# johannes-graeter/limo

Measured on AMD Instinct MI355X. Metric: keyframe-BA window solves/sec (5 KF, ~2k landmarks), higher is better.
Workload: dtype f64; 1 GPU; C2: KITTI-00-shaped windows, 5 keyframes x 2000 landmarks, LiDAR depth + ground plane, solveTrimmed schedule {2, trim 5%, <=100 LM iterations}; batch_windows_per_gpu=16384, distinct_windows_per_gpu=4096, observations_per_batch=144288124, depth_observations_per_batch=68405568, parallelism=single, converged=16328

## Files before the change

### limo_amd/csrc/kba_buffers.hpp

```cpp
#pragma once
#include <algorithm>
#include <cstddef>
#include <vector>

#include "kba_pack.hpp"

namespace kba {

template <typename F>
void for_each_buffer(const PackedBatch& P, BatchView& bv, F f) {
    bv.n_win = P.n_win;
    bv.TK = P.TK;
    bv.TL = P.TL;
    bv.TO = P.TO;
    bv.TV = P.TV;
    bv.TG = P.TG;
    bv.n_blk = P.n_blk;
    bv.n_lblk = P.n_lblk;
    bv.n_sblk = P.n_sblk;
    bv.Vmax = P.Vmax;
    bv.SO = P.SO;
    bv.SL = P.SL;
    bv.SG = P.SG;
    bv.SD = P.SD;
// ... 9 lines not shown
    KBA_BUF(win, NW * sizeof(WinDesc), P.win.data());
    KBA_BUF(st, NW * sizeof(WinState), nullptr);
    KBA_BUF(red, NW * sizeof(WinRed), nullptr);
    KBA_BUF(pose, TK * 7 * D, P.pose.data());
    KBA_BUF(pdir, TK * 3 * D, P.pdir.data());
    KBA_BUF(pdist, TK * D, P.pdist.data());
    KBA_BUF(lm, TL * 3 * D, P.lm.data());
    KBA_BUF(pose_c, TK * 7 * D, P.pose.data());
    KBA_BUF(pdir_c, TK * 3 * D, P.pdir.data());
    KBA_BUF(pdist_c, TK * D, P.pdist.data());
    KBA_BUF(lm_c, TL * 3 * D, P.lm.data());
    KBA_BUF(kf_win, TK * I, P.kf_win.data());
    KBA_BUF(kf_blk0, TK * I, P.kf_blk0.data());
    KBA_BUF(kf_nblk, TK * I, P.kf_nblk.data());
    KBA_BUF(kf_gp0, TK * I, P.kf_gp0.data());
    KBA_BUF(kf_ngp, TK * I, P.kf_ngp.data());
    KBA_BUF(cmask, TK * kCamSlots, P.cmask.data());
    KBA_BUF(cpresent, TK * kCamSlots, P.cpresent.data());
    KBA_BUF(cslot, TK * kCamSlots * I, P.cslot.data());
    KBA_BUF(lm_win, TL * I, P.lm_win.data());
    KBA_BUF(lm_id, TL * I, P.lm_id.data());
    KBA_BUF(lm_weight, TL * D, P.lm_weight.data());
    KBA_BUF(lm_state, TL, P.lm_state.data());
    KBA_BUF(lm_gp, TL * I, P.lm_gp.data());
    KBA_BUF(lm_slot, P.lm_slot.size() * I, P.lm_slot.data());
    KBA_BUF(view_kf, TV * I, P.view_kf.data());
    KBA_BUF(view_win, TV * I, P.view_win.data());
    KBA_BUF(view_cam, TV * 16 * D, P.view_cam.data());
    KBA_BUF(view_lin, TV * kViewLin * D, nullptr);
    KBA_BUF(view_lin_c, TV * kViewLin * D, nullptr);
    KBA_BUF(blk_view, NB * I, P.blk_view.data());
    KBA_BUF(blk_obs0, NB * I, P.blk_obs0.data());
    KBA_BUF(blk_n, NB * I, P.blk_n.data());
    KBA_BUF(obs_lm, TO * I, P.obs_lm.data());
    KBA_BUF(obs_u, TO * sizeof(float), P.obs_u.data());
    KBA_BUF(obs_v, TO * sizeof(float), P.obs_v.data());
    KBA_BUF(obs_d, TO * sizeof(float), P.obs_d.data());
    KBA_BUF(lblk_win, NL * I, P.lblk_win.data());
    KBA_BUF(lblk_lm0, NL * I, P.lblk_lm0.data());
    KBA_BUF(lblk_n, NL * I, P.lblk_n.data());
    KBA_BUF(sblk_win, NS * I, P.sblk_win.data());
    KBA_BUF(sblk_lm0, NS * I, P.sblk_lm0.data());
    KBA_BUF(sblk_n, NS * I, P.sblk_n.data());
    KBA_BUF(sgrp, NS * sizeof(SchurGroup), P.sgrp.empty() ? nullptr : P.sgrp.data());
    KBA_BUF(gp_lm, TG * I, P.gp_lm.data());
    KBA_BUF(gp_kf, TG * I, P.gp_kf.data());
    KBA_BUF(gp_w, TG * D, P.gp_w.data());
    KBA_BUF(gp_r, (size_t)P.SG * D, nullptr);
    KBA_BUF(gp_F, (size_t)P.SG * 10 * D, nullptr);
    KBA_BUF(gp_E, (size_t)P.SG * 3 * D, nullptr);
    KBA_BUF(gp_cost, TG * D, nullptr);
    KBA_BUF(gp_cost_c, TG * D, nullptr);
    KBA_BUF(obs_r, (size_t)(P.evaluate_only ? P.SO * 2 + P.SD : 1) * D, nullptr);
    KBA_BUF(obs_c, (size_t)(P.evaluate_only ? 1 : P.SO * 2) * D, nullptr);
    KBA_BUF(obs_Jp, (size_t)(P.evaluate_only ? P.SO * 12 + P.SD * 6 : 1) * D, nullptr);
    KBA_BUF(obs_Jl, (size_t)(P.evaluate_only ? P.SO * 6 + P.SD * 3 : 1) * D, nullptr);
    if (P.evaluate_only) KBA_BUF(echunk, (size_t)std::max(1, P.n_echunk) * sizeof(EvalChunk), P.echunk.empty() ? nullptr : P.echunk.data());
    KBA_BUF(lv_part, (size_t)(P.lvpart_total > 0 ? P.lvpart_total : 1) * D, nullptr);
    KBA_BUF(lblk_linfail, NL * D, nullptr);
    KBA_BUF(lm_V, (size_t)P.SL * 6 * D, nullptr);
    KBA_BUF(lm_g, (size_t)P.SL * 3 * D, nullptr);
    KBA_BUF(lm_scale, (size_t)P.SL * 3 * D, nullptr);
    KBA_BUF(lm_Li, (size_t)P.SL * 6 * D, nullptr);
    KBA_BUF(lblk_part, NL * 8 * D, nullptr);
    KBA_BUF(Hcc, (size_t)(P.hcc_total > 0 ? P.hcc_total : 1) * D, nullptr);
    KBA_BUF(gc, TK * kCamSlots * D, nullptr);
    KBA_BUF(scale_c, TK * kCamSlots * D, nullptr);
    KBA_BUF(yc, TK * kCamSlots * D, nullptr);
    KBA_BUF(delta_c, TK * kCamSlots * D, nullptr);
    KBA_BUF(S_part, (size_t)(P.spart_total > 0 ? P.spart_total : 1) * D, nullptr);
    KBA_BUF(S_red, (size_t)(P.sred_total > 0 ? P.sred_total : 1) * D, nullptr);
    KBA_BUF(cam_scratch, (size_t)(P.camscr_total > 0 ? P.camscr_total : 1) * D, nullptr);
    KBA_BUF(reg_cost, NW * 2 * D, nullptr);
    KBA_BUF(trim_rep, TL * D, nullptr);
    KBA_BUF(trim_dep, TL * D, nullptr);
    KBA_BUF(n_active, 8 * I, nullptr);
    if (P.n_shards > 1) {
        KBA_BUF(lblk_owner, NL * I, P.lblk_owner.data());
        KBA_BUF(gp_owner, TG * I, P.gp_owner.data());
    }
#undef KBA_BUF
}

inline ExchangeLayout exchange_layout(const PackedBatch& P) {
    ExchangeLayout L;
    auto pad = [](size_t n) { return (n + 31) / 32 * 32; };
    L.P = P.n_shards;
    L.n_win = P.n_win;
    L.TK = P.TK;
    L.n_lv = pad((size_t)std::max<int64_t>(1, P.xlv_total));
    L.n_w = pad((size_t)std::max(1, P.n_win));
    L.n_gp = pad((size_t)std::max(1, P.TK) * kGpRed);
    L.n_lb = pad((size_t)std::max(1, P.n_win) * 8);
    L.n_S = pad((size_t)std::max<int64_t>(1, P.sred_total / std::max(1, P.n_shards)));
    size_t o = 0;
    L.b_lv = o, o += L.n_lv;
    L.b_lf = o, o += L.n_w;
    L.b_gp = o, o += L.n_gp;
    L.b_gc = o, o += L.n_w;
    L.b_gcc = o, o += L.n_w;
    L.b_lb = o, o += L.n_lb;
    L.b_S = o, o += L.n_S;
    L.b_total = o;
    const size_t Pn = (size_t)L.P;
    o = 0;
    L.c_lv = o, o += Pn * L.n_lv;
    L.c_lf = o, o += Pn * L.n_w;
// ... 49 lines not shown
```

### limo_amd/csrc/kba_items.hpp

```cpp
#pragma once
#include "kba_layout.hpp"
#include "kba_lm.hpp"
#include "kba_math.hpp"

#ifndef KBA_SYNC
#define KBA_SYNC() ((void)0)
#endif
#if defined(KBA_PROFILE_TICKS) && defined(__HIPCC__)
__device__ long long kba_ticks[2][24];
#endif
#if defined(KBA_PROFILE_TICKS) && defined(__HIP_DEVICE_COMPILE__)
#define KBA_TICK(n)                                                                   \
    do {                                                                              \
        if (w == 0 && (tid == 0 || tid == nt - 1)) kba_ticks[tid != 0][n] = clock64(); \
    } while (0)
#else
#define KBA_TICK(n) ((void)0)
#endif

namespace kba {

struct LinLane {
    double e[kLinPartial];
    int fail;
// ... 270 lines not shown
        a.g[2] += e2 * r3[row];
    }
}
struct LmTailIn {
    int gg;
    int compute_scale;
    double radius;
    double sc[3];
};
KBA_HD void lin_lm_tail_fetch(const BatchView& bv, int w, int gl, LmTailIn& t) {
    t.gg = bv.lm_gp[gl];
    t.compute_scale = bv.st[w].compute_scale;
    t.radius = bv.st[w].radius;
    for (int i = 0; i < 3; ++i) t.sc[i] = t.compute_scale ? 1.0 : bv.lm_scale[i * bv.SL + gl];
}
KBA_HD void lin_lm_finish(const BatchView& bv, const SolveConsts& c, int gl, const double* x, const LmTailIn& t, LmAcc& a, double* part) {
    double* V = a.V;
    double* g = a.g;
    const int gg = t.gg;
    if (gg >= 0) {
        const double e0 = bv.gp_E[0 * bv.SG + gg], e1 = bv.gp_E[1 * bv.SG + gg], e2 = bv.gp_E[2 * bv.SG + gg];
        const double r = bv.gp_r[gg];
        V[0] += e0 * e0;
        V[1] += e0 * e1;
        V[2] += e0 * e2;
        V[3] += e1 * e1;
        V[4] += e1 * e2;
        V[5] += e2 * e2;
        g[0] += e0 * r;
        g[1] += e1 * r;
        g[2] += e2 * r;
    }
    for (int i = 0; i < 6; ++i) bv.lm_V[i * bv.SL + gl] = V[i];
    for (int i = 0; i < 3; ++i) bv.lm_g[i * bv.SL + gl] = g[i];
    double sc[3];
    if (t.compute_scale) {
        const double d[3] = {V[0], V[3], V[5]};
        for (int i = 0; i < 3; ++i) bv.lm_scale[i * bv.SL + gl] = sc[i] = c.jacobi_scaling ? 1.0 / (1.0 + sqrt(d[i])) : 1.0;
    } else {
        for (int i = 0; i < 3; ++i) sc[i] = t.sc[i];
    }
    part[0] = fmax(fabs(g[0]), fmax(fabs(g[1]), fabs(g[2])));
    part[1] = x[0] * x[0] + x[1] * x[1] + x[2] * x[2];
    part[5] = lm_damp_store(bv, c, t.radius, gl, sc, V, g) ? 1.0 : 0.0;
}
KBA_HD int lin_lm_lane(const BatchView& bv, const SolveConsts& c, int w, int gl, bool want_cost, LinLane* cam, double* part) {
    const WinDesc& wd = bv.win[w];
    part[0] = part[1] = part[5] = 0.0;
    for (int j = 0; j < wd.n_view; ++j) {
        cam[j].fail = 0;
        for (int i = 0; i < kLinPartial; ++i) cam[j].e[i] = 0.0;
    }
    const int state = bv.lm_state[gl];
    if (state == 0) return 0;
    LmAcc acc;
    for (int i = 0; i < 6; ++i) acc.V[i] = 0.0;
    for (int i = 0; i < 3; ++i) acc.g[i] = 0.0;
    int fail = 0;
    for (int j = 0; j < wd.n_view; ++j) {
        const int s = bv.lm_slot[(int64_t)j * bv.SL + gl];
        if (s < 0) continue;
        LinIn in;
        lin_fetch(bv, s, gl, in);
        const double* vl = bv.view_lin + (int64_t)kViewLin * (wd.view0 + j);
        double r3[3], c4[4];
        if (j < wd.n_view_fixed0) {
            if (!lin_obs<false>(vl, c, in, want_cost, r3, c4, cam[j])) fail = 1;
            if (state == 2) {
                cam[j].e[kLinFixedCost] = cam[j].e[0];
                cam[j].e[0] = 0.0;
            }
        } else {
            if (!lin_obs<true>(vl, c, in, want_cost, r3, c4, cam[j])) fail = 1;
            bv.obs_c[s] = c4[0];
            bv.obs_c[bv.SO + s] = c4[3];
        }
        lin_lm_accum(vl, r3, c4, acc);
    }
    if (state == 1) {
        LmTailIn t;
        lin_lm_tail_fetch(bv, w, gl, t);
        lin_lm_finish(bv, c, gl, bv.lm + 3 * (int64_t)gl, t, acc, part);
    }
    return fail;
}

KBA_HD void trim_residual_lane(const BatchView& bv, int b, int t, double* plane_rep, double* plane_dep) {
    if (t >= bv.blk_n[b]) return;
    const int view = bv.blk_view[b];
    const int64_t o = bv.blk_obs0[b] + t;
    const int gl = bv.obs_lm[o];
    double nr = -1.0, nd = -1.0;
    if (bv.lm_state[gl]) {
        const double* cam = bv.view_cam + 16 * (int64_t)view;
        double ruv[2], rd, zc[3];
        if (obs_residual(bv.pose + 7 * (int64_t)bv.view_kf[view], cam + 4, cam + 13, cam[0], cam[1], cam[2],
                         bv.lm + 3 * (int64_t)gl, bv.obs_u[o], bv.obs_v[o], bv.obs_d[o], ruv, &rd, zc)) {
            nr = sqrt(ruv[0] * ruv[0] + ruv[1] * ruv[1]);
        } else {
            nr = INFINITY;
        }
        if (bv.obs_d[o] > 0.0f) nd = fabs(zc[2] - static_cast<double>(bv.obs_d[o]));
    }
    plane_rep[o] = nr;
    plane_dep[o] = nd;
}

KBA_HD bool gp_row_fixed(const BatchView& bv, int g) {
    return bv.lm_state[bv.gp_lm[g]] == 2 && !bv.cmask[(int64_t)bv.gp_kf[g] * kCamSlots];
}
KBA_HD void gp_lane(const BatchView& bv, int g, bool candidate, double* cost_out) {
    const int gl = bv.gp_lm[g];
    const int gk = bv.gp_kf[g];
    GpOut o;
    const int state = bv.lm_state[gl];
    if (!state) {
        if (!candidate) {
            bv.gp_r[g] = 0.0;
            for (int i = 0; i < 10; ++i) bv.gp_F[i * bv.SG + g] = 0.0;
            for (int i = 0; i < 3; ++i) bv.gp_E[i * bv.SG + g] = 0.0;
        }
        cost_out[g] = 0.0;
        return;
    }
    if (candidate) {
        if (state == 2 && !bv.cmask[(int64_t)gk * kCamSlots]) {
            cost_out[g] = 0.0;
            return;
// ... 65 lines not shown
    double GB[9];
#pragma unroll
    for (int i = 0; i < 3; ++i) {
        GB[i * 3 + 0] = G[i * 3] * b00;
        GB[i * 3 + 1] = G[i * 3] * b01 + G[i * 3 + 1] * b11;
        GB[i * 3 + 2] = G[i * 3] * b02 + G[i * 3 + 1] * b12 + G[i * 3 + 2] * b22;
    }
#pragma unroll
    for (int a = 0; a < 3; ++a) {
#pragma unroll
        for (int cc = 0; cc < 3; ++cc) {
            const double yr = sc6[a] * (M[a] * GB[cc] + M[3 + a] * GB[3 + cc] + M[6 + a] * GB[6 + cc]);
            const double yt = sc6[3 + a] * GB[a * 3 + cc];
            Y[a * 3 + cc] = ASSIGN ? yr : Y[a * 3 + cc] + yr;
            Y[(3 + a) * 3 + cc] = ASSIGN ? yt : Y[(3 + a) * 3 + cc] + yt;
        }
    }
}

KBA_HD void schur_gp_block(const BatchView& bv, int gg, const uint8_t* cm, const double* lmk, const double* sc10, double* Y) {
    double E[3];
#pragma unroll
    for (int i = 0; i < 3; ++i) E[i] = bv.gp_E[i * bv.SG + gg];
    const double y0 = E[0] * lmk[0], y1 = E[0] * lmk[1] + E[1] * lmk[2], y2 = E[0] * lmk[3] + E[1] * lmk[4] + E[2] * lmk[5];
#pragma unroll
    for (int a = 0; a < kCamSlots; ++a) {
        if (!cm[a]) continue;
        const double f = bv.gp_F[a * bv.SG + gg] * sc10[a];
        Y[a * 3 + 0] += f * y0;
        Y[a * 3 + 1] += f * y1;
        Y[a * 3 + 2] += f * y2;
    }
}

KBA_HD void schur_pair_block(const BatchView& bv, const WinDesc& wd, int gl, int kl, const double* lmk, const double* sc,
                             const int* vkl, bool with_plane, double* Y) {
    for (int i = 0; i < 3 * kCamSlots; ++i) Y[i] = 0.0;
    const int row0 = kl * kCamSlots;
    const uint8_t* cm = bv.cmask + (int64_t)wd.cam0 + row0;
    if (cm[0]) {
        const double* pose = bv.pose + 7 * (int64_t)(wd.kf0 + kl);
        double R[9], M[9];
        bool have = false;
        for (int j = 0; j < wd.n_view; ++j) {
            if (vkl[j] != kl) continue;
            const int s = bv.lm_slot[(int64_t)j * bv.SL + gl];
            if (s < 0) continue;
            if (!have) {
                quat_R(pose, R);
                rot_tangent_from_R(R, quat_norm2_minus_1(pose), bv.lm + 3 * (int64_t)gl, M);
                have = true;
            }
            double Ft[9], c4[4];
            c4[0] = bv.obs_c[s];
            c4[3] = bv.obs_c[bv.SO + s];
            view_xy(bv.view_lin + (int64_t)kViewLin * (wd.view0 + j), bv.lm + 3 * (int64_t)gl, &c4[1], &c4[2]);
            ft_build(c4, bv.view_cam + 16 * (int64_t)(wd.view0 + j) + 4, Ft);
            schur_pose_block(Ft, R, M, lmk, sc + row0, Y);
        }
    }
    if (!with_plane) return;
    const int gg = bv.lm_gp[gl];
    if (gg < 0 || bv.gp_kf[gg] - wd.kf0 != kl) return;
    schur_gp_block(bv, gg, cm, lmk, sc + row0, Y);
}

KBA_HD void schur_load_lm(const BatchView& bv, int gl, double* lmk) {
#pragma unroll
    for (int i = 0; i < 6; ++i) lmk[i] = bv.lm_Li[i * bv.SL + gl];
}

KBA_HD int schur_plain_slabs(const WinDesc& wd, int span) { return (wd.n_sblk_plain + span - 1) / span; }
KBA_HD int schur_slabs(const WinDesc& wd, int span, int span_gp) {
    return schur_plain_slabs(wd, span) + (wd.n_sblk - wd.n_sblk_plain + span_gp - 1) / span_gp;
}
KBA_HD int schur_slab_of(const WinDesc& wd, int sb, int span, int span_gp) {
    const int i = sb - wd.sblk0;
    return i < wd.n_sblk_plain ? i / span : schur_plain_slabs(wd, span) + (i - wd.n_sblk_plain) / span_gp;
}
KBA_HD int schur_group_last(const WinDesc& wd, int sb, int span, int span_gp) {
    const int i = sb - wd.sblk0;
    const bool plain = i < wd.n_sblk_plain;
    const int end = plain ? wd.n_sblk_plain : wd.n_sblk, sp = plain ? span : span_gp;
    return wd.sblk0 + (i + sp < end ? i + sp : end) - 1;
}

KBA_HD int schur_need_count(int nf) { return nf * (nf + 1) / 2 + nf; }
KBA_HD int schur_need_pad(int nf) { return (schur_need_count(nf) + 31) / 32 * 32; }
KBA_HD void schur_need_decode(int i, int nf, int& ca, int& cb) {
    const int lda = nf + 1;
    ca = (int)(((2 * lda + 1) - sqrt((double)((2 * lda + 1) * (2 * lda + 1) - 8 * i))) * 0.5);
    while (ca > 0 && ca * lda - ca * (ca - 1) / 2 > i) --ca;
    while ((ca + 1) * lda - (ca + 1) * ca / 2 <= i) ++ca;
    cb = ca + (i - (ca * lda - ca * (ca - 1) / 2));
}
KBA_HD int schur_col(int i, int nfq);
KBA_HD int64_t schur_need_offset(int ca, int cb, int nf, int nfq, int nfp) {
    if (cb < nf) return (int64_t)schur_col(ca, nfq) * nfp + schur_col(cb, nfq);
    const int za = schur_col(ca, nfq);
    return za < nfq ? (int64_t)za * nfp + nfq : (int64_t)nfq * nfp + za;
}
KBA_HD void slab_reduce_entry(const BatchView& bv, int w, int n_shards, int i) {
    const WinDesc& wd = bv.win[w];
    const int64_t slab = (int64_t)wd.nf_pad * wd.nf_pad;
    int ca, cb;
    schur_need_decode(i, wd.nf, ca, cb);
    const double* sp = bv.S_part + wd.spart_off + schur_need_offset(ca, cb, wd.nf, wd.nfq, wd.nf_pad);
    double a = 0.0;
// ... 27 lines not shown
        g.kl[k] = on ? wd.fk[k] : -1;
        g.view[k] = on ? wd.fk_view[k] : -1;
        const int ci = on ? cslot[wd.cam0 + wd.fk[k] * kCamSlots] : -1;
        g.col0[k] = ci < 0 ? -1 : schur_col(ci, wd.nfq);
        g.pad2[k] = 0;
    }
    g.off_tile = wd.spart_off + (int64_t)g.q_slab * ((int64_t)wd.nf_pad * wd.nf_pad);
    g.off_packed = wd.spart_off + slab_packed_base(g.q_slab, schur_plain_slabs(wd, span), wd.nf, wd.nfq);
    return g;
}
KBA_HD int slab_packed_read(bool gp, int ca, int cb, int nf, int nfq) {
    if (gp) return schur_need_index(nf, ca, cb);
    if (ca >= nfq || (cb >= nfq && cb < nf)) return -1;
    return schur_need_index(nfq, ca, cb < nf ? cb : nfq);
}
KBA_HD int slab_packed_write(bool gp, int zr, int zc, int nf, int nfq) {
    const int n = gp ? nf : nfq;
    if (zr > zc || zc > n || (zr == nfq && zc == nfq)) return -1;
    if (zc == nfq) return schur_need_index(n, zr, n);
    if (zr == nfq) return schur_need_index(n, zc - 1, n);
    return schur_need_index(n, zr - (zr > nfq ? 1 : 0), zc - (zc > nfq ? 1 : 0));
}

struct LogProd {
    double m;
    int e;
};
KBA_HD void logprod_mul(LogProd& a, double x) {
    int ex;
    a.m *= frexp(x, &ex);
    a.e += ex;
}
KBA_HD double logprod_log(const LogProd& a) { return log(a.m) + static_cast<double>(a.e) * 0.69314718055994530942; }

KBA_HD void backsub_lane(const BatchView& bv, const SolveConsts& c, int w, int gl, double* part) {
    part[2] = part[3] = part[4] = part[6] = part[7] = 0.0;
    const int state = bv.lm_state[gl];
    const double* xp = bv.lm + 3 * (int64_t)gl;
    const double x[3] = {xp[0], xp[1], xp[2]};
    double xc[3] = {x[0], x[1], x[2]};
    if (state == 0) {
        double* o = bv.lm_c + 3 * (int64_t)gl;
        o[0] = xc[0];
        o[1] = xc[1];
        o[2] = xc[2];
        return;
    }
    const WinDesc& wd = bv.win[w];
    const int32_t* slot = bv.lm_slot + gl;
    const int n_view = wd.n_view;
    if (state == 1) {
        double a[3] = {0, 0, 0};
        const int j0 = wd.n_view_fixed0;
        int s_cur = j0 < n_view ? slot[(int64_t)j0 * bv.SL] : -1;
        int s_nxt = j0 + 1 < n_view ? slot[(int64_t)(j0 + 1) * bv.SL] : -1;
        double aun, sdn;
        {
            const int64_t o = s_cur >= 0 ? s_cur : 0;
            aun = bv.obs_c[o];
            sdn = bv.obs_c[bv.SO + o];
        }
        for (int j = j0; j < n_view; ++j) {
            const bool have = s_cur >= 0;
            double c4[4];
            c4[0] = have ? aun : 0.0;
            c4[3] = have ? sdn : 0.0;
            s_cur = s_nxt;
            s_nxt = j + 2 < n_view ? slot[(int64_t)(j + 2) * bv.SL] : -1;
            {
                const int64_t o = s_cur >= 0 ? s_cur : 0;
                aun = bv.obs_c[o];
                sdn = bv.obs_c[bv.SO + o];
            }
            const double* vs = bv.view_lin_c + (int64_t)kViewLin * (wd.view0 + j) + 28;
            const double* H = bv.view_lin + (int64_t)kViewLin * (wd.view0 + j);
            view_xy(H, x, &c4[1], &c4[2]);
            const double w0 = vs[0] * x[0] + vs[1] * x[1] + vs[2] * x[2] + vs[9];
            const double w1 = vs[3] * x[0] + vs[4] * x[1] + vs[5] * x[2] + vs[10];
            const double w2 = vs[6] * x[0] + vs[7] * x[1] + vs[8] * x[2] + vs[11];
            const double v0 = c4[0] * (c4[0] * (w0 - c4[1] * w2));
            const double v1 = c4[0] * (c4[0] * (w1 - c4[2] * w2));
            const double v2 = c4[3] * (c4[3] * w2) - c4[1] * v0 - c4[2] * v1;
            a[0] += H[0] * v0 + H[3] * v1 + H[6] * v2;
            a[1] += H[1] * v0 + H[4] * v1 + H[7] * v2;
            a[2] += H[2] * v0 + H[5] * v1 + H[8] * v2;
        }
        const int gg = bv.lm_gp[gl];
        if (gg >= 0) {
            const int gk = bv.gp_kf[gg];
            const double* dc = bv.delta_c + (int64_t)gk * kCamSlots;
            double q = 0.0;
            for (int k = 0; k < kCamSlots; ++k) q += bv.gp_F[k * bv.SG + gg] * dc[k];
            for (int cc = 0; cc < 3; ++cc) a[cc] += bv.gp_E[cc * bv.SG + gg] * q;
        }
        double Bt[6], t[3], V[6], g[3];
        for (int i = 0; i < 6; ++i) Bt[i] = bv.lm_Li[i * bv.SL + gl];
        for (int i = 0; i < 6; ++i) V[i] = bv.lm_V[i * bv.SL + gl];
        for (int i = 0; i < 3; ++i) g[i] = bv.lm_g[i * bv.SL + gl];
        lm_t_of(Bt, g, t);
        const double t0 = t[0] + Bt[0] * a[0];
        const double t1 = t[1] + Bt[1] * a[0] + Bt[2] * a[1];
        const double t2 = t[2] + Bt[3] * a[0] + Bt[4] * a[1] + Bt[5] * a[2];
        const double d0 = -(Bt[0] * t0 + Bt[1] * t1 + Bt[3] * t2);
        const double d1 = -(Bt[2] * t1 + Bt[4] * t2);
        const double d2 = -(Bt[5] * t2);
        xc[0] = x[0] + d0;
        xc[1] = x[1] + d1;
        xc[2] = x[2] + d2;
        const double Vd0 = V[0] * d0 + V[1] * d1 + V[2] * d2;
        const double Vd1 = V[1] * d0 + V[3] * d1 + V[4] * d2;
        const double Vd2 = V[2] * d0 + V[4] * d1 + V[5] * d2;
        part[2] = -(g[0] * d0 + g[1] * d1 + g[2] * d2) - (a[0] * d0 + a[1] * d1 + a[2] * d2) -
                  0.5 * (d0 * Vd0 + d1 * Vd1 + d2 * Vd2);
        const double e0 = x[0] - xc[0], e1 = x[1] - xc[1], e2 = x[2] - xc[2];
        part[3] = e0 * e0 + e1 * e1 + e2 * e2;
        part[4] = xc[0] * xc[0] + xc[1] * xc[1] + xc[2] * xc[2];
    }
    const double lw = bv.lm_weight[gl];
    const double c_rep = 1.0 / (c.a_rep * c.a_rep), c_dep = 1.0 / (c.a_dep * c.a_dep);
    LogProd lp_rep = {1.0, 0}, lp_dep = {1.0, 0};
    int fail = 0;
    const int j_prog = state == 2 ? wd.n_view_fixed0 : 0;
    {
        int s_cur = slot[0];
        int s_nxt = n_view > 1 ? slot[bv.SL] : -1;
        float un, vn, dn;
// ... 1140 lines not shown
```

### limo_amd/csrc/kba_kernels.hip

```cpp
#include <hip/hip_runtime.h>

#include <type_traits>

#define KBA_SYNC() __syncthreads()
#include "kba_items.hpp"

namespace kba {

__device__ __forceinline__ double wave_sum(double v) {
#pragma unroll
    for (int off = 32; off > 0; off >>= 1) v += __shfl_down(v, off, 64);
    return v;
}
__device__ __forceinline__ double wave_max(double v) {
#pragma unroll
    for (int off = 32; off > 0; off >>= 1) v = fmax(v, __shfl_down(v, off, 64));
    return v;
}

template <int N>
__device__ __forceinline__ void block_sum(const double* vals, double* lds , double* out_global) {
    const int lane = threadIdx.x & 63, wave = threadIdx.x >> 6;
#pragma unroll
    for (int i = 0; i < N; ++i) {
// ... 262 lines not shown
    const WinState& st = bv.st[bv.view_win[v]];
    if (!st.active || !st.need_lin) return;
    view_consts_item(bv, v);
}

typedef const double __attribute__((address_space(4))) cdouble;
constexpr int kLinAccl = 13;
constexpr int kLinVlds = 38;
template <bool VLDS>
__device__ __forceinline__ void lin_lm_block(const BatchView& bv, const SolveConsts& c, int b) {
    const int w = bv.lblk_win[b];
    const WinState& st = bv.st[w];
    if (!st.active || !st.need_lin) return;
    const bool want_cost = st.first != 0;
    const WinDesc& wd = bv.win[w];
    const int n_view = wd.n_view;
    const int n = bv.lblk_n[b];
    const int lane = threadIdx.x & 63, wave = threadIdx.x >> 6;
    const bool in_block = (int)threadIdx.x < n;
    const int gl = bv.lblk_lm0[b] + (in_block ? (int)threadIdx.x : n - 1);
    const int state = in_block ? bv.lm_state[gl] : 0;
    LinIn in;
    const bool take_candidate = st.accept != 0;
    const double* lm_src = take_candidate ? bv.lm_c : bv.lm;
    in.p[0] = lm_src[3 * (int64_t)gl];
    in.p[1] = lm_src[3 * (int64_t)gl + 1];
    in.p[2] = lm_src[3 * (int64_t)gl + 2];
    if (take_candidate && in_block) {
        bv.lm[3 * (int64_t)gl] = in.p[0];
        bv.lm[3 * (int64_t)gl + 1] = in.p[1];
        bv.lm[3 * (int64_t)gl + 2] = in.p[2];
    }
    in.w = bv.lm_weight[gl];
    in.sw = sqrt(in.w);
    LmTailIn tail;
    lin_lm_tail_fetch(bv, w, gl, tail);
    const int32_t* slot = bv.lm_slot + gl;
    double* out = bv.lv_part + wd.lvpart_off + (int64_t)(b - wd.lblk0) * n_view * kLinPartial;
    extern __shared__ __attribute__((aligned(16))) double lin_lds[];
    double* const vlds = lin_lds + kLinAccl * kBlock;
    double* const lv_lds = vlds + (VLDS ? n_view * kLinVlds : 0);
    double* const accl = lin_lds + threadIdx.x;
    typedef typename std::conditional<VLDS, const double*, cdouble*>::type VT;
    constexpr int kVStride = VLDS ? kLinVlds : kViewLin;
    VT vc;
    if constexpr (VLDS) {
        const double* src = bv.view_lin + (int64_t)kViewLin * wd.view0;
        for (int i = threadIdx.x; i < n_view * kLinVlds; i += kBlock) vlds[i] = src[(i / kLinVlds) * kViewLin + i % kLinVlds];
        __syncthreads();
        vc = vlds;
    } else {
        vc = (VT)(bv.view_lin + (int64_t)kViewLin * wd.view0);
    }
    const int64_t dump = bv.SO - kObsBlock + threadIdx.x;
#pragma unroll
    for (int i = 0; i < 9; ++i) accl[i * kBlock] = 0.0;
#pragma unroll
    for (int i = 0; i < 3; ++i) accl[(9 + i) * kBlock] = tail.sc[i];
    accl[12 * kBlock] = __hiloint2double(tail.gg, 0);
    auto accum = [&](auto vl, const double* r3, const double* c4) {
        LmAcc a;
#pragma unroll
        for (int i = 0; i < 6; ++i) a.V[i] = accl[i * kBlock];
#pragma unroll
        for (int i = 0; i < 3; ++i) a.g[i] = accl[(6 + i) * kBlock];
        lin_lm_accum(vl, r3, c4, a);
#pragma unroll
        for (int i = 0; i < 6; ++i) accl[i * kBlock] = a.V[i];
#pragma unroll
        for (int i = 0; i < 3; ++i) accl[(6 + i) * kBlock] = a.g[i];
    };
    int fail = 0;
    int s_cur = slot[0];
    int s_nxt = n_view > 1 ? slot[bv.SL] : -1;
    float u_n, v_n, d_n;
    {
        const int64_t o = s_cur >= 0 ? s_cur : 0;
        u_n = bv.obs_u[o];
        v_n = bv.obs_v[o];
        d_n = bv.obs_d[o];
    }
    const int rs14_idx = rs14_index(lane);
    const int j_cam0 = wd.n_view_fixed0;
    const int cost_slot = bv.lblk_lm0[b] - wd.lm0 >= wd.n_lm - wd.n_lm_const ? kLinFixedCost : 0;
    for (int j = 0; j < j_cam0; ++j) {
        VT vl = vc + (int64_t)j * kVStride;
        const int s = s_cur;
        in.u = u_n;
        in.v = v_n;
        in.d = d_n;
        s_cur = s_nxt;
        s_nxt = j + 2 < n_view ? slot[(int64_t)(j + 2) * bv.SL] : -1;
        {
            const int64_t o = s_cur >= 0 ? s_cur : 0;
            u_n = bv.obs_u[o];
            v_n = bv.obs_v[o];
            d_n = bv.obs_d[o];
        }
        const bool have = state != 0 && s >= 0;
        in.live = have;
        LinLane l;
        double r3[3], c4[4];
        if (!lin_obs<false>(vl, c, in, want_cost, r3, c4, l)) fail = 1;
        accum(vl, r3, c4);
        const double tot = wave_sum_all(l.e[0]);
        if (lane < kLinPartial) lv_lds[(j * kLinWaves + wave) * kLinPartial + lane] = lane == cost_slot ? tot : 0.0;
    }
    for (int j = j_cam0; j < n_view; ++j) {
        VT vl = vc + (int64_t)j * kVStride;
        const int s = s_cur;
        in.u = u_n;
        in.v = v_n;
        in.d = d_n;
        s_cur = s_nxt;
        s_nxt = j + 2 < n_view ? slot[(int64_t)(j + 2) * bv.SL] : -1;
        {
            const int64_t o = s_cur >= 0 ? s_cur : 0;
            u_n = bv.obs_u[o];
            v_n = bv.obs_v[o];
            d_n = bv.obs_d[o];
        }
        const bool have = state != 0 && s >= 0;
        in.live = have;
        LinLane l;
        double r3[3], c4[4];
        if (!lin_obs_core(vl, c, in, want_cost, r3, c4, l.e[0])) fail = 1;
        {
            const int64_t o = have ? s : dump;
            bv.obs_c[o] = c4[0];
            bv.obs_c[bv.SO + o] = c4[3];
        }
        accum(vl, r3, c4);
        static_assert(kLinPartial == 28 && kLinWaves * 64 == kBlock, "wave_reduce_scatter14 x 2");
        CamTmp ct;
        {
            double vals[14];
            lin_cam_half0(vl, in.p, c4, r3, l.e[0], ct, vals);
            const double tot = wave_reduce_scatter14(vals, lane);
            if (rs14_idx >= 0) lv_lds[(j * kLinWaves + wave) * kLinPartial + rs14_idx] = tot;
        }
        {
            double vals[14];
            lin_cam_half1(ct, vals);
            const double tot = wave_reduce_scatter14(vals, lane);
            if (rs14_idx >= 0) lv_lds[(j * kLinWaves + wave) * kLinPartial + 14 + rs14_idx] = tot;
        }
    }
    LmAcc acc;
#pragma unroll
    for (int i = 0; i < 6; ++i) acc.V[i] = accl[i * kBlock];
#pragma unroll
    for (int i = 0; i < 3; ++i) acc.g[i] = accl[(6 + i) * kBlock];
#pragma unroll
    for (int i = 0; i < 3; ++i) tail.sc[i] = accl[(9 + i) * kBlock];
    tail.gg = __double2hiint(accl[12 * kBlock]);
    double part[6] = {0.0, 0.0, 0.0, 0.0, 0.0, 0.0};
    if (in_block && tail.gg >= 0) gp_lane(bv, tail.gg, false, bv.gp_cost);
    if (state == 1) lin_lm_finish(bv, c, gl, in.p, tail, acc, part);
    __shared__ double lds[8];
    const double m = wave_max(part[0]);
    const double sm = wave_sum(part[1]);
    if (lane == 0) {
        lds[wave] = m;
        lds[4 + wave] = sm;
    }
    const int any_fail = __syncthreads_or(fail);
    const int any_damp_fail = __syncthreads_or(part[5] != 0.0);
    for (int e = threadIdx.x; e < n_view * kLinPartial; e += kBlock) {
        const double* q = lv_lds + (e / kLinPartial) * kLinWaves * kLinPartial + e % kLinPartial;
        out[e] = (q[0] + q[kLinPartial]) + (q[2 * kLinPartial] + q[3 * kLinPartial]);
    }
    if (threadIdx.x == 0) {
        bv.lblk_part[(int64_t)b * 8 + 0] = fmax(fmax(lds[0], lds[1]), fmax(lds[2], lds[3]));
        bv.lblk_part[(int64_t)b * 8 + 1] = (lds[4] + lds[5]) + (lds[6] + lds[7]);
        bv.lblk_part[(int64_t)b * 8 + 5] = any_damp_fail ? 1.0 : 0.0;
        bv.lblk_linfail[b] = any_fail ? 1.0 : 0.0;
    }
}
template <bool VLDS>
__global__ __launch_bounds__(kBlock) __attribute__((amdgpu_waves_per_eu(4, 4))) void k_lin_lm(BatchView bv, SolveConsts c, const int32_t* wl) {
    const int b = wl_at(bv, wl, blockIdx.x);
    if (b < 0) return;
    lin_lm_block<VLDS>(bv, c, b);
// ... 183 lines not shown
        __builtin_amdgcn_fence(__ATOMIC_RELEASE, "workgroup");
        __builtin_amdgcn_wave_barrier();
        __builtin_amdgcn_fence(__ATOMIC_ACQUIRE, "workgroup");
    } else {
        __syncthreads();
    }
}
template <int TM, bool GP, bool COOP>
__device__ __forceinline__ void schur_lean_group(const BatchView& bv, int sb, int span, int span_gp, int slab_packed, double* smem) {
    SchurGroup g;
    if (span == kSchurSpan && span_gp == kSchurSpanGp) {
        g = bv.sgrp[sb];
    } else {
        const int w = bv.sblk_win[sb];
        g = schur_group_make(bv.win[w], w, sb, span, span_gp, bv.sblk_lm0, bv.sblk_n, bv.cslot);
    }
    const int active = COOP ? 1 : __hip_atomic_load(&bv.st[g.w].active, __ATOMIC_RELAXED, __HIP_MEMORY_SCOPE_AGENT);
    const int nfq = g.nfq, nfp = g.nf_pad;
    const int ncol = GP ? g.nf + 1 : nfq + 1;
    const int ld = schur_lean_ld(ncol);
    const int Tt = (ncol + 15) / 16;
    constexpr bool kTT = !GP && TM == 2;
    const bool two_tile = kTT && Tt == 2;
    double* Z = smem;
    double* kc = Z + 3 * kSchurLm * ld + 16;
    int* zcs = reinterpret_cast<int*>(kc + 4 * kSpKf);
    const int lane = COOP ? (int)(threadIdx.x & 63) : (int)threadIdx.x, li = lane & 15, kq = lane >> 4;
    const int n_fk = g.n_fk;
    const int my_kl = kq == 0 ? g.kl[0] : kq == 1 ? g.kl[1] : kq == 2 ? g.kl[2] : g.kl[3];
    const int my_view = kq == 0 ? g.view[0] : kq == 1 ? g.view[1] : kq == 2 ? g.view[2] : g.view[3];
    const int my_col0 = kq == 0 ? g.col0[0] : kq == 1 ? g.col0[1] : kq == 2 ? g.col0[2] : g.col0[3];
    const bool have = my_col0 >= 0;
    const int slot0 = g.cam0 + (my_kl >= 0 ? my_kl : 0) * kCamSlots;
    const int32_t* my_slots = bv.lm_slot + (int64_t)(my_view >= 0 ? my_view - g.view0 : 0) * bv.SL;
    const int lm_first = g.lm_first, n_lm_blk = g.n_lm;

    constexpr int NT = (!GP && TM == 2) ? 2 : TM * (TM + 1) / 2;
    v4f64 acc[NT];
#pragma unroll
    for (int i = 0; i < NT; ++i) acc[i] = (v4f64){0.0, 0.0, 0.0, 0.0};

    auto index_issue = [&](int l0, int& st, int& slot, int& gr) {
        const int i = l0 + li < n_lm_blk ? l0 + li : n_lm_blk - 1;
        const int gl = lm_first + i;
        st = bv.lm_state[gl];
        slot = my_slots[gl];
        gr = -1;
        if constexpr (GP) gr = bv.lm_gp[gl];
    };
    auto index_kf = [&](int gr) {
        if constexpr (GP) return bv.gp_kf[gr >= 0 ? gr : 0];
        return 0;
    };
    auto index_mask = [&](int l0, int& st, int& slot, int& gg, int kf) {
        const bool in = l0 + li < n_lm_blk;
        st = in ? st : 0;
        slot = in && have && my_view >= 0 ? slot : -1;
        gg = GP && in && have && st == 1 && gg >= 0 && kf - g.kf0 == my_kl ? gg : -1;
    };
    double c4[4], p[3], Bt[6], g3[3], gE[3], gF[kCamSlots];
    bool live = false, seen = false, att = false;
    auto fetch_data = [&](int l0, int st, int slot, int gg) {
        const int gl = lm_first + l0 + li;
        live = st == 1;
        seen = live && slot >= 0;
        att = GP && live && gg >= 0;
        if (seen) {
            c4[0] = bv.obs_c[slot];
            c4[3] = bv.obs_c[bv.SO + slot];
#pragma unroll
            for (int i = 0; i < 3; ++i) p[i] = bv.lm[3 * (int64_t)gl + i];
        }
        const bool want_t = live && (kq == 0 || two_tile);
        if (seen || att || want_t) {
#pragma unroll
            for (int i = 0; i < 6; ++i) Bt[i] = bv.lm_Li[i * bv.SL + gl];
        }
        if (want_t) {
#pragma unroll
            for (int i = 0; i < 3; ++i) g3[i] = bv.lm_g[i * bv.SL + gl];
        }
        if constexpr (GP) {
            if (att) {
#pragma unroll
                for (int i = 0; i < 3; ++i) gE[i] = bv.gp_E[i * bv.SG + gg];
#pragma unroll
                for (int i = 0; i < kCamSlots; ++i) gF[i] = bv.gp_F[i * bv.SG + gg];
            }
        }
    };
    int n_st, n_slot, n_gg, n_kf;
    {
        int st0, sl0, gg0;
        index_issue(0, st0, sl0, gg0);
        index_issue(kSchurLm, n_st, n_slot, n_gg);
        const double* vl = bv.view_lin + (int64_t)kViewLin * (my_view >= 0 ? my_view : 0);
        const double v0 = vl[li], v1 = vl[16 + li], v2 = vl[32 + li];
        const int my_slot = slot0 + (li < kCamSlots ? li : 0);
        const double sc = bv.scale_c[my_slot];
        const int ci = bv.cslot[my_slot];
        const int kf_0 = index_kf(gg0);
        n_kf = index_kf(n_gg);
        index_mask(0, st0, sl0, gg0, kf_0);
        fetch_data(0, st0, sl0, gg0);
        if (!active) return;
        if (kq < n_fk) {
            double* mine_w = kc + kq * kSpKf;
            const bool vw = my_view >= 0;
            mine_w[li < 12 ? kSpH + li : kSpRc + li - 12] = vw ? v0 : 0.0;
            if (li < 5) mine_w[kSpRc + 4 + li] = vw ? v1 : 0.0;
            if (li >= 5 && li < 15) mine_w[li == 14 ? kSpQq1 : li - 5] = vw ? v2 : 0.0;
            if (li < kCamSlots) {
                mine_w[kSpScale + li] = sc;
                zcs[kq * 12 + li] = ci < 0 ? -1 : schur_col(ci, nfq);
            }
        }
        if (lane < 16) Z[3 * kSchurLm * ld + lane] = 0.0;
        schur_wave_sync<COOP>();
    }
    const double* mine = kc + (kq < n_fk ? kq : 0) * kSpKf;
    constexpr int NS = GP ? kCamSlots : 6;
    double yt[6] = {0.0, 0.0, 0.0, 0.0, 0.0, 0.0};
    const int mq = li < 8 ? li : li + 8;
    for (int l0 = 0; l0 < n_lm_blk; l0 += kSchurLm) {
        double t3[3] = {0.0, 0.0, 0.0};
        if (live && (kq == 0 || two_tile)) lm_t_of(Bt, g3, t3);
        if (kq == 0 && !two_tile) {
#pragma unroll
            for (int cc = 0; cc < 3; ++cc) Z[(3 * li + cc) * ld + nfq] = live ? t3[cc] : 0.0;
        }
        if (have) {
            double Y[3 * NS];
#pragma unroll
            for (int i = 0; i < 3 * NS; ++i) Y[i] = 0.0;
            if (seen) {
                double M[9], Ft[9];
                rot_tangent_from_R(mine, mine[kSpQq1], p, M);
                view_xy(mine + kSpH, p, &c4[1], &c4[2]);
                ft_build(c4, mine + kSpRc, Ft);
                schur_pose_block<true>(Ft, mine, M, Bt, mine + kSpScale, Y);
                if (two_tile) {
#pragma unroll
                    for (int a = 0; a < 6; ++a) yt[a] += Y[a * 3 + 0] * t3[0] + Y[a * 3 + 1] * t3[1] + Y[a * 3 + 2] * t3[2];
                }
            }
            if constexpr (GP) {
                if (att) {
                    const double y0 = gE[0] * Bt[0], y1 = gE[0] * Bt[1] + gE[1] * Bt[2], y2 = gE[0] * Bt[3] + gE[1] * Bt[4] + gE[2] * Bt[5];
#pragma unroll
                    for (int a = 0; a < kCamSlots; ++a) {
                        const double fa = zcs[kq * 12 + a] >= 0 ? gF[a] * mine[kSpScale + a] : 0.0;
                        Y[a * 3 + 0] += fa * y0;
                        Y[a * 3 + 1] += fa * y1;
                        Y[a * 3 + 2] += fa * y2;
                    }
                }
            }
            double* zrow = Z + 3 * li * ld + zcs[kq * 12];
#pragma unroll
            for (int a = 0; a < 6; ++a) {
                zrow[a] = Y[a * 3 + 0];
                zrow[ld + a] = Y[a * 3 + 1];
                zrow[2 * ld + a] = Y[a * 3 + 2];
            }
            if constexpr (GP) {
#pragma unroll
                for (int a = 6; a < kCamSlots; ++a) {
                    const int zc = zcs[kq * 12 + a];
                    if (zc >= 0) {
                        Z[(3 * li + 0) * ld + zc] = Y[a * 3 + 0];
                        Z[(3 * li + 1) * ld + zc] = Y[a * 3 + 1];
                        Z[(3 * li + 2) * ld + zc] = Y[a * 3 + 2];
                    }
                }
            }
        }
        {
            int st = n_st, slot = n_slot, gg = n_gg;
            index_mask(l0 + kSchurLm, st, slot, gg, n_kf);
            index_issue(l0 + 2 * kSchurLm, n_st, n_slot, n_gg);
            n_kf = index_kf(n_gg);
            fetch_data(l0 + kSchurLm, st, slot, gg);
        }
        schur_wave_sync<COOP>();
        const double* zp = Z + kq * ld + li;
        if (TM == 1 || Tt == 1) {
#pragma unroll
            for (int h = 0; h < 12; h += kSpBatch) {
                double pa[kSpBatch];
#pragma unroll
                for (int j = 0; j < kSpBatch; ++j) pa[j] = zp[(h + j) * 4 * ld];
#pragma unroll
                for (int j = 0; j < kSpBatch; ++j) acc[0] = __builtin_amdgcn_mfma_f64_16x16x4f64(pa[j], pa[j], acc[0], 0, 0, 0);
            }
        } else if (kTT) {
            if constexpr (kTT) {
                constexpr int kB = 3;
#pragma unroll
                for (int h = 0; h < 12; h += kB) {
                    double pa[kB], pb[kB], pq[kB];
#pragma unroll
                    for (int j = 0; j < kB; ++j) {
                        pa[j] = zp[(h + j) * 4 * ld];
                        pb[j] = zp[(h + j) * 4 * ld + 8];
                        pq[j] = Z[((h + j) * 4 + kq) * ld + mq];
                    }
#pragma unroll
                    for (int j = 0; j < kB; ++j) {
                        acc[0] = __builtin_amdgcn_mfma_f64_16x16x4f64(pa[j], pb[j], acc[0], 0, 0, 0);
                        acc[1] = __builtin_amdgcn_mfma_f64_16x16x4f64(pq[j], pq[j], acc[1], 0, 0, 0);
                    }
                }
            }
        } else if (TM == 2 || Tt == 2) {
            if constexpr (TM >= 2 && !kTT) {
                constexpr int i11 = TM;
#pragma unroll
                for (int h = 0; h < 12; h += kSpBatch) {
                    double pa[kSpBatch], pb[kSpBatch];
#pragma unroll
                    for (int j = 0; j < kSpBatch; ++j) {
                        pa[j] = zp[(h + j) * 4 * ld];
                        pb[j] = zp[(h + j) * 4 * ld + 16];
                    }
#pragma unroll
                    for (int j = 0; j < kSpBatch; ++j) {
                        acc[0] = __builtin_amdgcn_mfma_f64_16x16x4f64(pa[j], pa[j], acc[0], 0, 0, 0);
                        acc[1] = __builtin_amdgcn_mfma_f64_16x16x4f64(pa[j], pb[j], acc[1], 0, 0, 0);
                        acc[i11] = __builtin_amdgcn_mfma_f64_16x16x4f64(pb[j], pb[j], acc[i11], 0, 0, 0);
                    }
                }
            }
        } else {
            if constexpr (TM >= 3) {
#pragma unroll
// ... 896 lines not shown
```

### limo_amd/csrc/kba_layout.hpp

```cpp
#pragma once
#include <stddef.h>
#include <stdint.h>

#include "../../include/limo_hip.h"

namespace kba {

constexpr int kMaxKf = 20;
constexpr int kMaxViews = 64;
constexpr int kViewLin = 64;
constexpr int kCamSlots = 10;
constexpr int kMaxNc = kMaxKf * kCamSlots;
constexpr int kBlock = 256;
constexpr int kObsPerLane = 4;
constexpr int kObsBlock = kBlock * kObsPerLane;
constexpr int kSchurLm = 16;
constexpr int kSchurLmPerBlock = 64;
constexpr int kSchurSpan = 2, kSchurSpanGp = 1;
constexpr int kMaxRegRows = 1 + (kMaxKf - 1) * 5 + 3 * kMaxKf;

constexpr int kGpRed = 65;
constexpr int kLinPartial = 28;
constexpr int kLinFixedCost = 26;
constexpr int kLinWaves = 4;
// ... 143 lines not shown
    const int32_t* lblk_win;
    const int32_t* lblk_lm0;
    const int32_t* lblk_n;
    const int32_t* sblk_win;
    const int32_t* sblk_lm0;
    const int32_t* sblk_n;
    const SchurGroup* sgrp;
    const int32_t* lblk_owner;
    const int32_t* gp_owner;
    double* x_lv;
    double* x_lf;
    double* x_gp;
    double* x_gc;
    double* x_gcc;
    double* x_lb;
    const double* gp_red;
    int32_t gp_red_P, pad_x;
    const int32_t* gp_lm;
    const int32_t* gp_kf;
    const double* gp_w;
    double *gp_r, *gp_F, *gp_E;
    double* gp_cost;
    double* gp_cost_c;
    double *obs_r, *obs_c;
    double *obs_Jp, *obs_Jl;
    const EvalChunk* echunk;
    int64_t SD;
    int32_t n_echunk, pad_e;
    double* lv_part;
    double* lblk_linfail;
    double *lm_V, *lm_g;
    double *lm_scale;
    double* lm_Li;
    double* lblk_part;
    double *Hcc, *gc;
    double *scale_c, *yc, *delta_c;
    double *S_part;
    double *S_red;
    double* cam_scratch;
    double* reg_cost;
    double *trim_rep, *trim_dep;
    int32_t* n_active;
    int32_t* n_active_host;
    int32_t counted;
    int32_t n_slots;
    int32_t* slot_win;
    int32_t* sched_ctl;
    int32_t* slot_cnt;
    int32_t* sched_lists;
    int32_t sched_off[SL_COUNT];
    int32_t* sched_done_host;
};

struct ExchangeLayout {
    int P = 1, n_win = 0, TK = 0;
    size_t n_lv = 0, n_w = 0, n_gp = 0, n_lb = 0, n_S = 0;
    size_t b_lv = 0, b_lf = 0, b_gp = 0, b_gc = 0, b_gcc = 0, b_lb = 0, b_S = 0, b_total = 0;
    size_t c_lv = 0, c_lf = 0, c_gp = 0, c_gc = 0, c_gcc = 0, c_lb = 0, c_S = 0, c_total = 0;
    size_t trim_count = 0;
    size_t spart_count = 1;
#if defined(__HIPCC__)
    __host__ __device__
#endif
    void range(int point, size_t& off, size_t& count) const {
        off = point == 2 ? b_S : point == 4 ? b_gcc : 0;
        const size_t end = point == 1 || point == 4 ? b_S : b_total;
        count = end - off;
    }
};

}
```

Baseline: 37720 windows/s.

## Store per-observation cost coefficients in landmark-major view planes

The per-observation cost terms (obs_c) move from observation-slot indexing to a [view][landmark] plane layout, sized by Vmax*SL. Consumers in the Schur and back-substitution kernels can then read them with coalesced, landmark-contiguous loads, with no indirect slot lookup and no dump-slot writes. The Schur loop prefetch is also restructured: index and data issues are split, and the ground-plane path is software-pipelined separately from the plain path. In exchange the buffer grows to cover unused (view, landmark) pairs, and missing pairs are now explicitly zeroed, which adds writes.

```diff
diff --git a/limo_amd/csrc/kba_buffers.hpp b/limo_amd/csrc/kba_buffers.hpp
--- a/limo_amd/csrc/kba_buffers.hpp
+++ b/limo_amd/csrc/kba_buffers.hpp
@@ -85,7 +85,7 @@
     KBA_BUF(gp_cost, TG * D, nullptr);
     KBA_BUF(gp_cost_c, TG * D, nullptr);
     KBA_BUF(obs_r, (size_t)(P.evaluate_only ? P.SO * 2 + P.SD : 1) * D, nullptr);
-    KBA_BUF(obs_c, (size_t)(P.evaluate_only ? 1 : P.SO * 2) * D, nullptr);
+    KBA_BUF(obs_c, (P.evaluate_only ? 1 : P.lm_slot.size() * 2) * D, nullptr);
     KBA_BUF(obs_Jp, (size_t)(P.evaluate_only ? P.SO * 12 + P.SD * 6 : 1) * D, nullptr);
     KBA_BUF(obs_Jl, (size_t)(P.evaluate_only ? P.SO * 6 + P.SD * 3 : 1) * D, nullptr);
     if (P.evaluate_only) KBA_BUF(echunk, (size_t)std::max(1, P.n_echunk) * sizeof(EvalChunk), P.echunk.empty() ? nullptr : P.echunk.data());
diff --git a/limo_amd/csrc/kba_items.hpp b/limo_amd/csrc/kba_items.hpp
--- a/limo_amd/csrc/kba_items.hpp
+++ b/limo_amd/csrc/kba_items.hpp
@@ -346,6 +346,8 @@
         for (int i = 0; i < kLinPartial; ++i) cam[j].e[i] = 0.0;
     }
     const int state = bv.lm_state[gl];
+    const int64_t PS = obs_c_stride(bv);
+    for (int j = wd.n_view_fixed0; j < wd.n_view; ++j) bv.obs_c[(int64_t)j * bv.SL + gl] = bv.obs_c[PS + (int64_t)j * bv.SL + gl] = 0.0;
     if (state == 0) return 0;
     LmAcc acc;
     for (int i = 0; i < 6; ++i) acc.V[i] = 0.0;
@@ -366,8 +368,8 @@
             }
         } else {
             if (!lin_obs<true>(vl, c, in, want_cost, r3, c4, cam[j])) fail = 1;
-            bv.obs_c[s] = c4[0];
-            bv.obs_c[bv.SO + s] = c4[3];
+            bv.obs_c[(int64_t)j * bv.SL + gl] = c4[0];
+            bv.obs_c[PS + (int64_t)j * bv.SL + gl] = c4[3];
         }
         lin_lm_accum(vl, r3, c4, acc);
     }
@@ -539,8 +541,8 @@
                 have = true;
             }
             double Ft[9], c4[4];
-            c4[0] = bv.obs_c[s];
-            c4[3] = bv.obs_c[bv.SO + s];
+            c4[0] = bv.obs_c[(int64_t)j * bv.SL + gl];
+            c4[3] = bv.obs_c[obs_c_stride(bv) + (int64_t)j * bv.SL + gl];
             view_xy(bv.view_lin + (int64_t)kViewLin * (wd.view0 + j), bv.lm + 3 * (int64_t)gl, &c4[1], &c4[2]);
             ft_build(c4, bv.view_cam + 16 * (int64_t)(wd.view0 + j) + 4, Ft);
             schur_pose_block(Ft, R, M, lmk, sc + row0, Y);
@@ -674,26 +676,25 @@
     if (state == 1) {
         double a[3] = {0, 0, 0};
         const int j0 = wd.n_view_fixed0;
-        int s_cur = j0 < n_view ? slot[(int64_t)j0 * bv.SL] : -1;
-        int s_nxt = j0 + 1 < n_view ? slot[(int64_t)(j0 + 1) * bv.SL] : -1;
-        double aun, sdn;
-        {
-            const int64_t o = s_cur >= 0 ? s_cur : 0;
-            aun = bv.obs_c[o];
-            sdn = bv.obs_c[bv.SO + o];
+        const double* au_p = bv.obs_c;
+        const double* sd_p = au_p + obs_c_stride(bv);
+        int64_t r = (int64_t)j0 * bv.SL + gl;
+        int s_cur = -1;
+        double aun = 0.0, sdn = 0.0;
+        if (j0 < n_view) {
+            s_cur = bv.lm_slot[r];
+            aun = au_p[r];
+            sdn = sd_p[r];
         }
         for (int j = j0; j < n_view; ++j) {
             const bool have = s_cur >= 0;
             double c4[4];
             c4[0] = have ? aun : 0.0;
             c4[3] = have ? sdn : 0.0;
-            s_cur = s_nxt;
-            s_nxt = j + 2 < n_view ? slot[(int64_t)(j + 2) * bv.SL] : -1;
-            {
-                const int64_t o = s_cur >= 0 ? s_cur : 0;
-                aun = bv.obs_c[o];
-                sdn = bv.obs_c[bv.SO + o];
-            }
+            r += j + 1 < n_view ? bv.SL : 0;
+            s_cur = bv.lm_slot[r];
+            aun = au_p[r];
+            sdn = sd_p[r];
             const double* vs = bv.view_lin_c + (int64_t)kViewLin * (wd.view0 + j) + 28;
             const double* H = bv.view_lin + (int64_t)kViewLin * (wd.view0 + j);
             view_xy(H, x, &c4[1], &c4[2]);
diff --git a/limo_amd/csrc/kba_kernels.hip b/limo_amd/csrc/kba_kernels.hip
--- a/limo_amd/csrc/kba_kernels.hip
+++ b/limo_amd/csrc/kba_kernels.hip
@@ -338,7 +338,8 @@
     } else {
         vc = (VT)(bv.view_lin + (int64_t)kViewLin * wd.view0);
     }
-    const int64_t dump = bv.SO - kObsBlock + threadIdx.x;
+    double* const plane = bv.obs_c + gl;
+    const int64_t plane_stride = obs_c_stride(bv);
 #pragma unroll
     for (int i = 0; i < 9; ++i) accl[i * kBlock] = 0.0;
 #pragma unroll
@@ -412,9 +413,10 @@
         double r3[3], c4[4];
         if (!lin_obs_core(vl, c, in, want_cost, r3, c4, l.e[0])) fail = 1;
         {
-            const int64_t o = have ? s : dump;
-            bv.obs_c[o] = c4[0];
-            bv.obs_c[bv.SO + o] = c4[3];
+            if (in_block) {
+                plane[(int64_t)j * bv.SL] = have ? c4[0] : 0.0;
+                plane[plane_stride + (int64_t)j * bv.SL] = c4[3];
+            }
         }
         accum(vl, r3, c4);
         static_assert(kLinPartial == 28 && kLinWaves * 64 == kBlock, "wave_reduce_scatter14 x 2");
@@ -704,57 +706,61 @@
         if constexpr (GP) return bv.gp_kf[gr >= 0 ? gr : 0];
         return 0;
     };
-    auto index_mask = [&](int l0, int& st, int& slot, int& gg, int kf) {
+    double c4[4], p[3], Bt[6], g3[3], gE[3], gF[kCamSlots];
+    const bool has_pair = have && my_view >= 0;
+    const bool want_g = kq == 0 || two_tile;
+    const double* my_au = bv.obs_c + (int64_t)(my_view >= 0 ? my_view - g.view0 : 0) * bv.SL;
+    const double* my_sd = my_au + obs_c_stride(bv);
+    auto data_issue = [&](int l0) {
+        const int gl = lm_first + (l0 + li < n_lm_blk ? l0 + li : n_lm_blk - 1);
+        if (has_pair) {
+            c4[0] = my_au[gl];
+            c4[3] = my_sd[gl];
+#pragma unroll
+            for (int i = 0; i < 3; ++i) p[i] = bv.lm[3 * (int64_t)gl + i];
+        }
+        if (has_pair || want_g || (GP && have)) {
+#pragma unroll
+            for (int i = 0; i < 6; ++i) Bt[i] = bv.lm_Li[i * bv.SL + gl];
+        }
+        if (want_g) {
+#pragma unroll
+            for (int i = 0; i < 3; ++i) g3[i] = bv.lm_g[i * bv.SL + gl];
+        }
+    };
+    auto gp_issue = [&](bool on, int gg) {
+        if constexpr (GP) {
+            if (on) {
+#pragma unroll
+                for (int i = 0; i < 3; ++i) gE[i] = bv.gp_E[i * bv.SG + gg];
+#pragma unroll
+                for (int i = 0; i < kCamSlots; ++i) gF[i] = bv.gp_F[i * bv.SG + gg];
+            }
+        }
+    };
+    bool live = false, seen = false, att = false;
+    auto predicates = [&](int l0, int st, int slot, int gg, int kf) {
         const bool in = l0 + li < n_lm_blk;
-        st = in ? st : 0;
-        slot = in && have && my_view >= 0 ? slot : -1;
-        gg = GP && in && have && st == 1 && gg >= 0 && kf - g.kf0 == my_kl ? gg : -1;
+        live = in && st == 1;
+        seen = live && has_pair && slot >= 0;
+        att = GP && live && have && gg >= 0 && kf - g.kf0 == my_kl;
     };
-    double c4[4], p[3], Bt[6], g3[3], gE[3], gF[kCamSlots];
-    bool live = false, seen = false, att = false;
-    auto fetch_data = [&](int l0, int st, int slot, int gg) {
-        const int gl = lm_first + l0 + li;
-        live = st == 1;
-        seen = live && slot >= 0;
-        att = GP && live && gg >= 0;
-        if (seen) {
-            c4[0] = bv.obs_c[slot];
-            c4[3] = bv.obs_c[bv.SO + slot];
-#pragma unroll
-            for (int i = 0; i < 3; ++i) p[i] = bv.lm[3 * (int64_t)gl + i];
-        }
-        const bool want_t = live && (kq == 0 || two_tile);
-        if (seen || att || want_t) {
-#pragma unroll
-            for (int i = 0; i < 6; ++i) Bt[i] = bv.lm_Li[i * bv.SL + gl];
-        }
-        if (want_t) {
-#pragma unroll
-            for (int i = 0; i < 3; ++i) g3[i] = bv.lm_g[i * bv.SL + gl];
-        }
-        if constexpr (GP) {
-            if (att) {
-#pragma unroll
-                for (int i = 0; i < 3; ++i) gE[i] = bv.gp_E[i * bv.SG + gg];
-#pragma unroll
-                for (int i = 0; i < kCamSlots; ++i) gF[i] = bv.gp_F[i * bv.SG + gg];
-            }
-        }
-    };
-    int n_st, n_slot, n_gg, n_kf;
+    int c_st, c_slot, c_gg, c_kf = 0;
+    int n_st = 0, n_slot = -1, n_gg = -1, n_kf = 0;
     {
-        int st0, sl0, gg0;
-        index_issue(0, st0, sl0, gg0);
-        index_issue(kSchurLm, n_st, n_slot, n_gg);
+        index_issue(0, c_st, c_slot, c_gg);
+        if constexpr (GP) index_issue(kSchurLm, n_st, n_slot, n_gg);
         const double* vl = bv.view_lin + (int64_t)kViewLin * (my_view >= 0 ? my_view : 0);
         const double v0 = vl[li], v1 = vl[16 + li], v2 = vl[32 + li];
         const int my_slot = slot0 + (li < kCamSlots ? li : 0);
         const double sc = bv.scale_c[my_slot];
         const int ci = bv.cslot[my_slot];
-        const int kf_0 = index_kf(gg0);
-        n_kf = index_kf(n_gg);
-        index_mask(0, st0, sl0, gg0, kf_0);
-        fetch_data(0, st0, sl0, gg0);
+        data_issue(0);
+        if constexpr (GP) {
+            c_kf = index_kf(c_gg);
+            n_kf = index_kf(n_gg);
+            gp_issue(have && li < n_lm_blk && c_gg >= 0, c_gg);
+        }
         if (!active) return;
         if (kq < n_fk) {
             double* mine_w = kc + kq * kSpKf;
@@ -775,6 +781,7 @@
     double yt[6] = {0.0, 0.0, 0.0, 0.0, 0.0, 0.0};
     const int mq = li < 8 ? li : li + 8;
     for (int l0 = 0; l0 < n_lm_blk; l0 += kSchurLm) {
+        predicates(l0, c_st, c_slot, c_gg, c_kf);
         double t3[3] = {0.0, 0.0, 0.0};
         if (live && (kq == 0 || two_tile)) lm_t_of(Bt, g3, t3);
         if (kq == 0 && !two_tile) {
@@ -827,12 +834,18 @@
                 }
             }
         }
-        {
-            int st = n_st, slot = n_slot, gg = n_gg;
-            index_mask(l0 + kSchurLm, st, slot, gg, n_kf);
-            index_issue(l0 + 2 * kSchurLm, n_st, n_slot, n_gg);
-            n_kf = index_kf(n_gg);
-            fetch_data(l0 + kSchurLm, st, slot, gg);
+        if (l0 + kSchurLm < n_lm_blk) {
+            const int l1 = l0 + kSchurLm;
+            if constexpr (GP) {
+                c_st = n_st, c_slot = n_slot, c_gg = n_gg, c_kf = n_kf;
+                index_issue(l1 + kSchurLm, n_st, n_slot, n_gg);
+                n_kf = index_kf(n_gg);
+                data_issue(l1);
+                gp_issue(have && l1 + li < n_lm_blk && c_st == 1 && c_gg >= 0 && c_kf - g.kf0 == my_kl, c_gg);
+            } else {
+                index_issue(l1, c_st, c_slot, c_gg);
+                data_issue(l1);
+            }
         }
         schur_wave_sync<COOP>();
         const double* zp = Z + kq * ld + li;
diff --git a/limo_amd/csrc/kba_layout.hpp b/limo_amd/csrc/kba_layout.hpp
--- a/limo_amd/csrc/kba_layout.hpp
+++ b/limo_amd/csrc/kba_layout.hpp
@@ -219,6 +219,11 @@
     int32_t* sched_done_host;
 };
 
+#if defined(__HIPCC__)
+__host__ __device__
+#endif
+inline int64_t obs_c_stride(const BatchView& bv) { return (int64_t)(bv.Vmax > 0 ? bv.Vmax : 1) * bv.SL; }
+
 struct ExchangeLayout {
     int P = 1, n_win = 0, TK = 0;
     size_t n_lv = 0, n_w = 0, n_gp = 0, n_lb = 0, n_S = 0;
```

After: 38160 windows/s (median of 6 runs). +1.2%, better.
